# opendilab/DI-hpc

Measured on AMD Instinct MI355X. Metric: gae_fwd_bwd_samples_per_sec, higher is better.
Workload: dtype f32; 1 GPU; GAE fwd+bwd, T=1024, global B=65536 (65536 per GPU), fp32 (BASELINE.json configs[1]); T=1024, B_per_gpu=65536, global_B=65536, parallelism=batch-sharded x1, no data-path collective, launch=eager

## Files before the change

### di-hpc_amd/csrc/gae.hip

```cpp
#include <hip/hip_runtime.h>
#include <hip/hip_ext.h>

#include <atomic>
#include <initializer_list>
#include <new>
#include <type_traits>

#include "hostutil.hpp"
#include "hpc_rll_hip.h"
#include "wave.hpp"

namespace hpc_rll {
namespace {

__device__ __forceinline__ double geom_sum(double lam, int k) {
    if (k <= 0) return 0.0;
    if (lam == 1.0) return (double)k;
    if (lam > 0.0) return -expm1((double)k * log(lam)) / (1.0 - lam);
    return (1.0 - pow(lam, (double)k)) / (1.0 - lam);
}

__global__ void gae_coef_kernel(float* __restrict__ coef, int T, float gamma, float lambda) {
    const int t = blockIdx.x * blockDim.x + threadIdx.x;
    if (t >= T) return;
    const int k = T - t;
    const double lam = (double)lambda;
    coef[t] = (float)((double)gamma * lam * geom_sum(lam, k - 1) / geom_sum(lam, k));
}

template <int V, int LC, int NW, bool NTL, bool NTS, bool HALF = false>
__global__ __launch_bounds__(NW * 64) void gae_fwd_kernel(const float* __restrict__ value,
                                                          const float* __restrict__ reward,
                                                          float* __restrict__ adv,
                                                          const float* __restrict__ coef, int T, int B,
                                                          float gamma) {
    static_assert(!HALF || V == 1, "half-wave tiles hold one column per lane");
    constexpr int NWV = HALF ? 2 * NW : NW;
    constexpr int TILE = HALF ? 32 : 64 * V;
    __shared__ float lds[2 * NWV * TILE + 2 * NWV];
    float* const s_l0 = lds;
    float* const s_p0 = lds + 2 * NWV * TILE;

    const int lane = threadIdx.x & 63;
    const int wr = __builtin_amdgcn_readfirstlane((int)(threadIdx.x >> 6));
    const int cl = HALF ? (lane & 31) : lane;
    const int w = HALF ? 2 * wr + (lane >> 5) : wr;
    const long col = (long)blockIdx.x * TILE + (long)cl * V;
    const bool col_ok = col < (long)B;

    float carry[V];
#pragma unroll
    for (int k = 0; k < V; ++k) carry[k] = 0.f;

    constexpr int SPAN = NWV * LC;
    const int n_iter = (T + SPAN - 1) / SPAN;

    for (int it = 0; it < n_iter; ++it) {
        const int t1 = T - (it * NWV + (NWV - 1 - w)) * LC;
        const int t0 = t1 - LC;
        const int buf = it & 1;

        float L[LC][V];
        float P[LC];

        if (t0 >= 0) {
            Pack<V> vr[LC + 1], rr[LC];
            if (col_ok) {
                const float* vp = value + (size_t)t0 * B + col;
                const float* rp = reward + (size_t)t0 * B + col;
#pragma unroll
                for (int j = LC; j >= 0; --j) vr[j] = load_pack<V, NTL>(vp + (size_t)j * B);
#pragma unroll
                for (int j = LC - 1; j >= 0; --j) rr[j] = load_pack<V, NTL>(rp + (size_t)j * B);
            } else {
#pragma unroll
                for (int j = 0; j <= LC; ++j)
#pragma unroll
                    for (int k = 0; k < V; ++k) vr[j].v[k] = 0.f;
#pragma unroll
                for (int j = 0; j < LC; ++j)
#pragma unroll
                    for (int k = 0; k < V; ++k) rr[j].v[k] = 0.f;
            }
            float a[V];
#pragma unroll
            for (int k = 0; k < V; ++k) a[k] = 0.f;
            float p = 1.f;
#pragma unroll
            for (int j = LC - 1; j >= 0; --j) {
                const float c = coef[t0 + j];
#pragma unroll
                for (int k = 0; k < V; ++k) {
                    const float delta = fmaf(gamma, vr[j + 1].v[k], rr[j].v[k]) - vr[j].v[k];
                    a[k] = fmaf(c, a[k], delta);
                    L[j][k] = a[k];
                }
                p *= c;
                P[j] = p;
            }
        } else {
            float a[V];
#pragma unroll
            for (int k = 0; k < V; ++k) a[k] = 0.f;
            float p = 1.f;
#pragma unroll
            for (int j = LC - 1; j >= 0; --j) {
                const int t = t0 + j;
                if (t >= 0) {
                    const float c = coef[t];
                    Pack<V> v0, v1, r;
                    if (col_ok) {
                        v0 = load_pack<V, NTL>(value + (size_t)t * B + col);
                        v1 = load_pack<V, NTL>(value + (size_t)(t + 1) * B + col);
                        r = load_pack<V, NTL>(reward + (size_t)t * B + col);
                    } else {
#pragma unroll
                        for (int k = 0; k < V; ++k) v0.v[k] = v1.v[k] = r.v[k] = 0.f;
                    }
#pragma unroll
                    for (int k = 0; k < V; ++k) {
                        const float delta = fmaf(gamma, v1.v[k], r.v[k]) - v0.v[k];
                        a[k] = fmaf(c, a[k], delta);
                    }
                    p *= c;
                }
#pragma unroll
                for (int k = 0; k < V; ++k) L[j][k] = a[k];
                P[j] = p;
            }
        }

#pragma unroll
        for (int k = 0; k < V; ++k) s_l0[(buf * NWV + w) * TILE + cl * V + k] = L[0][k];
        if (cl == 0) s_p0[buf * NWV + w] = P[0];
        __syncthreads();

        float A[V], Aw[V];
#pragma unroll
        for (int k = 0; k < V; ++k) { A[k] = carry[k]; Aw[k] = 0.f; }
#pragma unroll
        for (int u = NWV - 1; u >= 0; --u) {
            if (u == w) {
#pragma unroll
                for (int k = 0; k < V; ++k) Aw[k] = A[k];
            }
            const float p0 = s_p0[buf * NWV + u];
#pragma unroll
            for (int k = 0; k < V; ++k) A[k] = fmaf(p0, A[k], s_l0[(buf * NWV + u) * TILE + cl * V + k]);
        }
#pragma unroll
        for (int k = 0; k < V; ++k) carry[k] = A[k];

        if (col_ok) {
#pragma unroll
            for (int j = LC - 1; j >= 0; --j) {
                const int t = t0 + j;
                if (t >= 0) {
                    Pack<V> o;
#pragma unroll
                    for (int k = 0; k < V; ++k) o.v[k] = fmaf(P[j], Aw[k], L[j][k]);
                    store_pack<V, NTS>(adv + (size_t)t * B + col, o);
                }
            }
        }
    }
}

template <int V, int LC, int NW, bool NTL, bool NTS, bool FULLB>
__global__ __launch_bounds__(NW * 64) void gae_fwd_pf_kernel(const float* __restrict__ value,
                                                             const float* __restrict__ reward,
                                                             float* __restrict__ adv,
                                                             const float* __restrict__ coef, int T, int B,
                                                             float gamma) {
    constexpr int TILE = 64 * V;
    __shared__ float lds[2 * NW * TILE + 2 * NW];
    float* const s_l0 = lds;
    float* const s_p0 = lds + 2 * NW * TILE;

    const int lane = threadIdx.x & 63;
    const int w = __builtin_amdgcn_readfirstlane((int)(threadIdx.x >> 6));
    const long col = (long)blockIdx.x * TILE + (long)lane * V;
    const bool col_ok = FULLB || col < (long)B;

    float carry[V];
#pragma unroll
    for (int k = 0; k < V; ++k) carry[k] = 0.f;

    constexpr int SPAN = NW * LC;
    const int n_full = T / SPAN;
    const bool ragged = (T % SPAN) != 0;

    Pack<V> vr[LC + 1], rr[LC];
#pragma unroll
    for (int j = 0; j <= LC; ++j)
#pragma unroll
        for (int k = 0; k < V; ++k) vr[j].v[k] = 0.f;
#pragma unroll
    for (int j = 0; j < LC; ++j)
#pragma unroll
        for (int k = 0; k < V; ++k) rr[j].v[k] = 0.f;

    auto chunk_t0 = [&](int it) { return T - (it * NW + (NW - 1 - w)) * LC - LC; };
    auto issue = [&](int it) {
        if (col_ok) {
            const int t0 = chunk_t0(it);
            const float* vp = value + (size_t)t0 * B + col;
            const float* rp = reward + (size_t)t0 * B + col;
#pragma unroll
            for (int j = LC; j >= 0; --j) vr[j] = load_pack<V, NTL>(vp + (size_t)j * B);
#pragma unroll
            for (int j = LC - 1; j >= 0; --j) rr[j] = load_pack<V, NTL>(rp + (size_t)j * B);
        }
    };
    auto finish = [&](auto guard_, int it, int t0, float (&L)[LC][V], float (&P)[LC]) {
        constexpr bool GUARD = decltype(guard_)::value != 0;
        const int buf = it & 1;
#pragma unroll
        for (int k = 0; k < V; ++k) s_l0[(buf * NW + w) * TILE + lane * V + k] = L[0][k];
        if (lane == 0) s_p0[buf * NW + w] = P[0];
        __syncthreads();
        float A[V], Aw[V];
#pragma unroll
        for (int k = 0; k < V; ++k) { A[k] = carry[k]; Aw[k] = 0.f; }
#pragma unroll
        for (int u = NW - 1; u >= 0; --u) {
            if (u == w) {
#pragma unroll
                for (int k = 0; k < V; ++k) Aw[k] = A[k];
            }
            const float p0 = s_p0[buf * NW + u];
#pragma unroll
            for (int k = 0; k < V; ++k) A[k] = fmaf(p0, A[k], s_l0[(buf * NW + u) * TILE + lane * V + k]);
        }
#pragma unroll
        for (int k = 0; k < V; ++k) carry[k] = A[k];
        if (col_ok) {
#pragma unroll
            for (int j = LC - 1; j >= 0; --j) {
                const int t = t0 + j;
                if (!GUARD || t >= 0) {
                    Pack<V> o;
#pragma unroll
                    for (int k = 0; k < V; ++k) o.v[k] = fmaf(P[j], Aw[k], L[j][k]);
                    store_pack<V, NTS>(adv + (size_t)t * B + col, o);
                }
            }
        }
    };

    if (n_full > 0) issue(0);
    for (int it = 0; it < n_full; ++it) {
        const int t0 = chunk_t0(it);
        float L[LC][V];
        float P[LC];
        {
            float a[V];
#pragma unroll
            for (int k = 0; k < V; ++k) a[k] = 0.f;
            float p = 1.f;
#pragma unroll
            for (int j = LC - 1; j >= 0; --j) {
                const float c = coef[t0 + j];
#pragma unroll
                for (int k = 0; k < V; ++k) {
                    const float delta = fmaf(gamma, vr[j + 1].v[k], rr[j].v[k]) - vr[j].v[k];
                    a[k] = fmaf(c, a[k], delta);
                    L[j][k] = a[k];
                }
                p *= c;
                P[j] = p;
            }
        }
        if (it + 1 < n_full) issue(it + 1);
        finish(std::integral_constant<int, 0>{}, it, t0, L, P);
    }
    if (ragged) {
        const int it = n_full;
        const int t0 = chunk_t0(it);
        float L[LC][V];
        float P[LC];
        float a[V];
#pragma unroll
        for (int k = 0; k < V; ++k) a[k] = 0.f;
        float p = 1.f;
#pragma unroll
        for (int j = LC - 1; j >= 0; --j) {
            const int t = t0 + j;
            if (t >= 0) {
                const float c = coef[t];
                Pack<V> v0, v1, r;
                if (col_ok) {
                    v0 = load_pack<V, NTL>(value + (size_t)t * B + col);
                    v1 = load_pack<V, NTL>(value + (size_t)(t + 1) * B + col);
                    r = load_pack<V, NTL>(reward + (size_t)t * B + col);
                } else {
#pragma unroll
                    for (int k = 0; k < V; ++k) v0.v[k] = v1.v[k] = r.v[k] = 0.f;
                }
#pragma unroll
                for (int k = 0; k < V; ++k) {
                    const float delta = fmaf(gamma, v1.v[k], r.v[k]) - v0.v[k];
                    a[k] = fmaf(c, a[k], delta);
                }
                p *= c;
            }
#pragma unroll
            for (int k = 0; k < V; ++k) L[j][k] = a[k];
            P[j] = p;
        }
        finish(std::integral_constant<int, 1>{}, it, t0, L, P);
    }
}

template <int V, int LC, int NW, bool NTL, bool NTS, bool HALF = false>
__global__ __launch_bounds__(NW * 64) void gae_bwd_kernel(const float* __restrict__ grad_adv,
                                                          float* __restrict__ grad_value,
                                                          float* __restrict__ grad_reward,
                                                          const float* __restrict__ coef, int T, int B,
                                                          float gamma) {
    static_assert(!HALF || V == 1, "half-wave tiles hold one column per lane");
    constexpr int NWV = HALF ? 2 * NW : NW;
    constexpr int TILE = HALF ? 32 : 64 * V;
    __shared__ float lds[2 * NWV * TILE + 2 * NWV];
    float* const s_l0 = lds;
    float* const s_p0 = lds + 2 * NWV * TILE;

    const int lane = threadIdx.x & 63;
    const int wr = __builtin_amdgcn_readfirstlane((int)(threadIdx.x >> 6));
    const int cl = HALF ? (lane & 31) : lane;
    const int w = HALF ? 2 * wr + (lane >> 5) : wr;
    const long col = (long)blockIdx.x * TILE + (long)cl * V;
    const bool col_ok = col < (long)B;

    float carry[V];
#pragma unroll
    for (int k = 0; k < V; ++k) carry[k] = 0.f;

    constexpr int SPAN = NWV * LC;
    const int n_iter = (T + SPAN - 1) / SPAN;

    for (int it = 0; it < n_iter; ++it) {
        const int t0 = (it * NWV + w) * LC;
        const int buf = it & 1;

        float L[LC][V];
        float Q[LC];
        {
            float a[V];
#pragma unroll
            for (int k = 0; k < V; ++k) a[k] = 0.f;
            float q = 1.f;
            if (t0 + LC <= T) {
                Pack<V> g[LC];
                if (col_ok) {
                    const float* gp = grad_adv + (size_t)t0 * B + col;
#pragma unroll
                    for (int j = 0; j < LC; ++j) g[j] = load_pack<V, NTL>(gp + (size_t)j * B);
                } else {
#pragma unroll
                    for (int j = 0; j < LC; ++j)
#pragma unroll
                        for (int k = 0; k < V; ++k) g[j].v[k] = 0.f;
                }
#pragma unroll
                for (int j = 0; j < LC; ++j) {
                    const int t = t0 + j;
                    const float c = (t > 0) ? coef[t - 1] : 0.f;
#pragma unroll
                    for (int k = 0; k < V; ++k) {
                        a[k] = fmaf(c, a[k], g[j].v[k]);
                        L[j][k] = a[k];
                    }
                    q *= c;
                    Q[j] = q;
                }
            } else {
#pragma unroll
                for (int j = 0; j < LC; ++j) {
                    const int t = t0 + j;
                    if (t < T) {
                        const float c = (t > 0) ? coef[t - 1] : 0.f;
                        Pack<V> g;
                        if (col_ok) {
                            g = load_pack<V, NTL>(grad_adv + (size_t)t * B + col);
                        } else {
#pragma unroll
                            for (int k = 0; k < V; ++k) g.v[k] = 0.f;
                        }
#pragma unroll
                        for (int k = 0; k < V; ++k) a[k] = fmaf(c, a[k], g.v[k]);
                        q *= c;
                    }
#pragma unroll
                    for (int k = 0; k < V; ++k) L[j][k] = a[k];
                    Q[j] = q;
                }
            }
        }

#pragma unroll
        for (int k = 0; k < V; ++k) s_l0[(buf * NWV + w) * TILE + cl * V + k] = L[LC - 1][k];
        if (cl == 0) s_p0[buf * NWV + w] = Q[LC - 1];
        __syncthreads();

        float A[V], Aw[V];
#pragma unroll
        for (int k = 0; k < V; ++k) { A[k] = carry[k]; Aw[k] = 0.f; }
#pragma unroll
        for (int u = 0; u < NWV; ++u) {
            if (u == w) {
#pragma unroll
                for (int k = 0; k < V; ++k) Aw[k] = A[k];
            }
            const float q0 = s_p0[buf * NWV + u];
#pragma unroll
            for (int k = 0; k < V; ++k) A[k] = fmaf(q0, A[k], s_l0[(buf * NWV + u) * TILE + cl * V + k]);
        }
#pragma unroll
        for (int k = 0; k < V; ++k) carry[k] = A[k];

        if (col_ok) {
            float prev[V];
#pragma unroll
            for (int k = 0; k < V; ++k) prev[k] = Aw[k];
#pragma unroll
            for (int j = 0; j < LC; ++j) {
                const int t = t0 + j;
                if (t < T) {
                    Pack<V> d, gv;
#pragma unroll
                    for (int k = 0; k < V; ++k) {
                        d.v[k] = fmaf(Q[j], Aw[k], L[j][k]);
                        gv.v[k] = fmaf(gamma, prev[k], -d.v[k]);
                        prev[k] = d.v[k];
                    }
                    if (grad_reward) store_pack<V, NTS>(grad_reward + (size_t)t * B + col, d);
                    if (grad_value) {
                        store_pack<V, NTS>(grad_value + (size_t)t * B + col, gv);
                        if (t == T - 1) {
                            Pack<V> last;
#pragma unroll
                            for (int k = 0; k < V; ++k) last.v[k] = gamma * d.v[k];
                            store_pack<V, NTS>(grad_value + (size_t)T * B + col, last);
                        }
                    }
                }
            }
        }
    }
}

template <int V, int LC, int NW, bool NTL, bool NTS, bool FULLB>
__global__ __launch_bounds__(NW * 64) void gae_bwd_pf_kernel(const float* __restrict__ grad_adv,
                                                             float* __restrict__ grad_value,
                                                             float* __restrict__ grad_reward,
                                                             const float* __restrict__ coef, int T, int B,
                                                             float gamma) {
    constexpr int TILE = 64 * V;
    __shared__ float lds[2 * NW * TILE + 2 * NW];
    float* const s_l0 = lds;
    float* const s_p0 = lds + 2 * NW * TILE;

    const int lane = threadIdx.x & 63;
    const int w = __builtin_amdgcn_readfirstlane((int)(threadIdx.x >> 6));
    const long col = (long)blockIdx.x * TILE + (long)lane * V;
    const bool col_ok = FULLB || col < (long)B;

    float carry[V];
#pragma unroll
    for (int k = 0; k < V; ++k) carry[k] = 0.f;

    constexpr int SPAN = NW * LC;
    const int n_full = T / SPAN;
    const bool ragged = (T % SPAN) != 0;

    Pack<V> g[LC];
#pragma unroll
    for (int j = 0; j < LC; ++j)
#pragma unroll
        for (int k = 0; k < V; ++k) g[j].v[k] = 0.f;

    auto chunk_t0 = [&](int it) { return (it * NW + w) * LC; };
    auto issue = [&](int it) {
        if (col_ok) {
            const float* gp = grad_adv + (size_t)chunk_t0(it) * B + col;
#pragma unroll
            for (int j = 0; j < LC; ++j) g[j] = load_pack<V, NTL>(gp + (size_t)j * B);
        }
    };
    auto finish = [&](auto guard_, int it, int t0, float (&L)[LC][V], float (&Q)[LC]) {
        constexpr bool GUARD = decltype(guard_)::value != 0;
        const int buf = it & 1;
#pragma unroll
        for (int k = 0; k < V; ++k) s_l0[(buf * NW + w) * TILE + lane * V + k] = L[LC - 1][k];
        if (lane == 0) s_p0[buf * NW + w] = Q[LC - 1];
        __syncthreads();
        float A[V], Aw[V];
#pragma unroll
        for (int k = 0; k < V; ++k) { A[k] = carry[k]; Aw[k] = 0.f; }
#pragma unroll
        for (int u = 0; u < NW; ++u) {
            if (u == w) {
#pragma unroll
                for (int k = 0; k < V; ++k) Aw[k] = A[k];
            }
            const float q0 = s_p0[buf * NW + u];
#pragma unroll
            for (int k = 0; k < V; ++k) A[k] = fmaf(q0, A[k], s_l0[(buf * NW + u) * TILE + lane * V + k]);
        }
#pragma unroll
        for (int k = 0; k < V; ++k) carry[k] = A[k];
        if (col_ok) {
            float prev[V];
#pragma unroll
            for (int k = 0; k < V; ++k) prev[k] = Aw[k];
#pragma unroll
            for (int j = 0; j < LC; ++j) {
                const int t = t0 + j;
                if (!GUARD || t < T) {
                    Pack<V> d, gv;
#pragma unroll
                    for (int k = 0; k < V; ++k) {
                        d.v[k] = fmaf(Q[j], Aw[k], L[j][k]);
                        gv.v[k] = fmaf(gamma, prev[k], -d.v[k]);
                        prev[k] = d.v[k];
                    }
                    store_pack<V, NTS>(grad_reward + (size_t)t * B + col, d);
                    store_pack<V, NTS>(grad_value + (size_t)t * B + col, gv);
                    if ((GUARD || j == LC - 1) && t == T - 1) {
                        Pack<V> last;
#pragma unroll
                        for (int k = 0; k < V; ++k) last.v[k] = gamma * d.v[k];
                        store_pack<V, NTS>(grad_value + (size_t)T * B + col, last);
                    }
                }
            }
        }
    };

    if (n_full > 0) issue(0);
    for (int it = 0; it < n_full; ++it) {
        const int t0 = chunk_t0(it);
        float L[LC][V];
        float Q[LC];
        {
            float a[V];
#pragma unroll
            for (int k = 0; k < V; ++k) a[k] = 0.f;
            float q = 1.f;
#pragma unroll
            for (int j = 0; j < LC; ++j) {
                const int t = t0 + j;
                const float c = (t > 0) ? coef[t - 1] : 0.f;
#pragma unroll
                for (int k = 0; k < V; ++k) {
                    a[k] = fmaf(c, a[k], g[j].v[k]);
                    L[j][k] = a[k];
                }
                q *= c;
                Q[j] = q;
            }
        }
        if (it + 1 < n_full) issue(it + 1);
        finish(std::integral_constant<int, 0>{}, it, t0, L, Q);
    }
    if (ragged) {
        const int it = n_full;
        const int t0 = chunk_t0(it);
        float L[LC][V];
        float Q[LC];
        float a[V];
#pragma unroll
        for (int k = 0; k < V; ++k) a[k] = 0.f;
        float q = 1.f;
#pragma unroll
        for (int j = 0; j < LC; ++j) {
            const int t = t0 + j;
            if (t < T) {
                const float c = (t > 0) ? coef[t - 1] : 0.f;
                Pack<V> gg;
                if (col_ok) {
                    gg = load_pack<V, NTL>(grad_adv + (size_t)t * B + col);
                } else {
#pragma unroll
                    for (int k = 0; k < V; ++k) gg.v[k] = 0.f;
                }
#pragma unroll
                for (int k = 0; k < V; ++k) a[k] = fmaf(c, a[k], gg.v[k]);
                q *= c;
            }
#pragma unroll
            for (int k = 0; k < V; ++k) L[j][k] = a[k];
            Q[j] = q;
        }
        finish(std::integral_constant<int, 1>{}, it, t0, L, Q);
    }
}

struct Cfg { int v, lc, nw, flags; bool half; bool pf; bool pf_refused; int plain_flags; };

struct KTime {
    bool on = false;
    int cap = 0, n = 0;
    hipEvent_t* ev = nullptr;
    int* kind = nullptr;
    std::atomic<int> last_cfg[2][6] = {};
};
KTime g_kt;

template <class K, class... A>
inline void launch(K kernel, dim3 grid, dim3 block, hipStream_t st, int kind, A... args) {
    if (g_kt.on && g_kt.n < g_kt.cap) {
        const int i = g_kt.n++;
        g_kt.kind[i] = kind;
        hipExtLaunchKernelGGL(kernel, grid, block, 0, st, g_kt.ev[2 * i], g_kt.ev[2 * i + 1], 0, args...);
    } else {
        hipLaunchKernelGGL(kernel, grid, block, 0, st, args...);
    }
}

inline int max_vec(int B, std::initializer_list<const void*> ptrs) {
    for (int v : {4, 2}) {
        bool ok = (B % v) == 0;
        for (const void* p : ptrs) ok = ok && aligned(p, 4 * v);
        if (ok) return v;
    }
    return 1;
}

inline Cfg choose_cfg(bool fwd, int T, int B, int vmax, int v, int lc, int nw, int flags) {
    auto wgs_for = [&](int vv) { return (B + 64 * vv - 1) / (64 * vv); };
    const bool all_auto = v == 0 && lc == 0 && nw == 0;
    const bool all_explicit = v != 0 && lc != 0 && nw != 0;
    const bool streaming = (12.0 * (double)T * (double)B) >= 300e6;
    int av, alc, anw, afl;
    bool apf = false;
    if (streaming && fwd) {
        av = (B >= 65536 && vmax >= 2) ? 2 : 1;
        const int wgs = wgs_for(av);
        if (wgs >= 1024) { alc = 16; anw = 8; }
        else if (wgs >= 512) { alc = 8; anw = av == 2 ? 2 : 4; }
        else { alc = 16; anw = 8; }
        afl = 3;
        if (vmax >= 2) {
            if (B < 65536) { if (B >= 32768) { av = 2; alc = 16; anw = 8; apf = true; } }
            else if (B < 131072) {
                if (vmax >= 4) { av = 4; alc = 4; anw = 8; } else { av = 2; alc = 4; anw = 4; }
                apf = true;
            }
            else if (B >= 262144) { av = 2; alc = 16; anw = 4; apf = true; }
        }
    } else if (streaming) {
        if (B >= 262144) { av = 1; alc = 8; anw = 8; apf = true; }
        else if (B >= 65536 && vmax >= 4) { av = 4; alc = 2; anw = 4; apf = true; }
        else if (B >= 131072 && vmax >= 2) { av = 2; alc = 2; anw = 4; }
        else if (B >= 65536 && vmax >= 2) { av = 2; alc = 2; anw = 4; }
        else if (B >= 32768 && vmax >= 4) { av = 4; alc = 4; anw = 4; apf = true; }
        else { av = 1; alc = 8; anw = 8; }
        afl = 2;
    } else {
        av = 1; alc = 16; anw = 4;
        while (anw < 16 && wgs_for(1) * anw < 2048) anw <<= 1;
        afl = 2;
        if (T >= 512 && wgs_for(1) >= 256 && anw == 8) {
            apf = true;
            if (!fwd) alc = 8;
        }
    }
    if (v == 0) v = av;
    if (v > vmax) v = vmax;
    if (lc == 0) {
        lc = alc;
        if (lc == 16 && v == 4) lc = 8;
    }
    if (nw == 0) {
        nw = anw;
        const int chunks = (T + lc - 1) / lc;
        while (nw > 1 && nw > chunks) nw >>= 1;
    }
    const int explicit_flags = flags;
    bool half = flags >= 0 && (flags & 4);
    if (flags < 0) {
        flags = afl;
        half = all_auto && !streaming && v == 1 && lc == 16 && nw == 16 && wgs_for(1) < 256 && T >= 512;
    }
    if (half && !(v == 1 && nw == 16 && (lc == 8 || lc == 16))) half = false;
    bool pf = !half && (explicit_flags >= 0 ? (explicit_flags & 8) != 0 : (all_auto && apf));
    if (pf && !(nw == 2 || nw == 4 || nw == 8)) pf = false;
    if (pf && fwd && !((lc == 4 || lc == 8 || lc == 16) && !(v == 4 && lc == 16) && !(v == 1 && lc == 4))) pf = false;
    if (pf && !fwd && !((lc == 2 || lc == 4 || lc == 8) && !(v == 1 && lc != 8))) pf = false;
    const int plain_flags = flags & 3;
    if (pf) flags |= 2;
    const bool pf_asked = explicit_flags >= 0 && (explicit_flags & 8) != 0;
    const bool pf_refused = pf_asked && (!all_explicit || (!half && !pf));
    Cfg out{v, lc, nw, flags & 3, half, pf, pf_refused, plain_flags};
    return out;
}

template <int N> using I = std::integral_constant<int, N>;

template <class F>
inline void for_each_cfg(F&& f) {
#define HPC_RLL_NW_ROW(V, LC) \
    f(I<V>{}, I<LC>{}, I<1>{}); f(I<V>{}, I<LC>{}, I<2>{}); f(I<V>{}, I<LC>{}, I<4>{}); \
    f(I<V>{}, I<LC>{}, I<8>{}); f(I<V>{}, I<LC>{}, I<16>{});
    HPC_RLL_NW_ROW(1, 4) HPC_RLL_NW_ROW(1, 8) HPC_RLL_NW_ROW(1, 16)
    HPC_RLL_NW_ROW(2, 2) HPC_RLL_NW_ROW(2, 4) HPC_RLL_NW_ROW(2, 8) HPC_RLL_NW_ROW(2, 16)
    HPC_RLL_NW_ROW(4, 2) HPC_RLL_NW_ROW(4, 4) HPC_RLL_NW_ROW(4, 8)
#undef HPC_RLL_NW_ROW
}

#define HPC_RLL_GAE_DISPATCH(KERNEL, KIND, ...)                                                    \
    do {                                                                                           \
        bool hit = false;                                                                          \
        {                                                                                          \
            std::atomic<int>* lc_ = g_kt.last_cfg[KIND];                                           \
            lc_[0] = cfg.v; lc_[1] = cfg.lc; lc_[2] = cfg.nw; lc_[3] = cfg.flags; lc_[4] = cfg.half; lc_[5] = cfg.pf; \
        }                                                                                          \
        if (cfg.half) {                                                                            \
            const dim3 grid((unsigned)((B + 31) / 32)), block(1024);                               \
            const bool ntl = cfg.flags & 1;                                                        \
            if (cfg.lc == 16) {                                                                    \
                if (ntl) launch(KERNEL<1, 16, 16, true, true, true>, grid, block, st, KIND, __VA_ARGS__);   \
                else launch(KERNEL<1, 16, 16, false, true, true>, grid, block, st, KIND, __VA_ARGS__);      \
            } else {                                                                               \
                if (ntl) launch(KERNEL<1, 8, 16, true, true, true>, grid, block, st, KIND, __VA_ARGS__);    \
                else launch(KERNEL<1, 8, 16, false, true, true>, grid, block, st, KIND, __VA_ARGS__);       \
            }                                                                                      \
            hit = true;                                                                            \
        }                                                                                          \
        auto go = [&](auto V_, auto LC_, auto NW_) {                                               \
            constexpr int V = decltype(V_)::value, LC = decltype(LC_)::value,                      \
                          NW = decltype(NW_)::value;                                               \
            if (!hit && cfg.v == V && cfg.lc == LC && cfg.nw == NW) {                                \
                const dim3 grid((unsigned)((B + 64 * V - 1) / (64 * V))), block(NW * 64);          \
                switch (cfg.flags) {                                                               \
                    case 0: launch(KERNEL<V, LC, NW, false, false>, grid, block, st, KIND, __VA_ARGS__); break; \
                    case 1: launch(KERNEL<V, LC, NW, true, false>, grid, block, st, KIND, __VA_ARGS__); break;  \
                    case 2: launch(KERNEL<V, LC, NW, false, true>, grid, block, st, KIND, __VA_ARGS__); break;  \
                    default: launch(KERNEL<V, LC, NW, true, true>, grid, block, st, KIND, __VA_ARGS__); break;  \
                }                                                                                  \
                hit = true;                                                                        \
            }                                                                                      \
        };                                                                                         \
        for_each_cfg(go);                                                                          \
        if (!hit) return HPC_RLL_EUNSUPPORTED;                                                     \
    } while (0)

template <class... A>
inline bool dispatch_fwd_pf(const Cfg& cfg, int B, hipStream_t st, A... args) {
    bool hit = false;
    auto go = [&](auto V_, auto LC_, auto NW_) {
        constexpr int V = decltype(V_)::value, LC = decltype(LC_)::value, NW = decltype(NW_)::value;
        if (!hit && cfg.v == V && cfg.lc == LC && cfg.nw == NW) {
            const dim3 grid((unsigned)((B + 64 * V - 1) / (64 * V))), block(NW * 64);
            const bool full = (B % (64 * V)) == 0;
            if (cfg.flags & 1) {
                if (full) launch(gae_fwd_pf_kernel<V, LC, NW, true, true, true>, grid, block, st, 0, args...);
                else launch(gae_fwd_pf_kernel<V, LC, NW, true, true, false>, grid, block, st, 0, args...);
            } else {
                if (full) launch(gae_fwd_pf_kernel<V, LC, NW, false, true, true>, grid, block, st, 0, args...);
                else launch(gae_fwd_pf_kernel<V, LC, NW, false, true, false>, grid, block, st, 0, args...);
            }
            hit = true;
        }
    };
#define HPC_RLL_PF_ROW(V, LC) go(I<V>{}, I<LC>{}, I<2>{}); go(I<V>{}, I<LC>{}, I<4>{}); go(I<V>{}, I<LC>{}, I<8>{});
    HPC_RLL_PF_ROW(1, 8) HPC_RLL_PF_ROW(1, 16) HPC_RLL_PF_ROW(2, 4) HPC_RLL_PF_ROW(2, 8) HPC_RLL_PF_ROW(2, 16)
    HPC_RLL_PF_ROW(4, 4) HPC_RLL_PF_ROW(4, 8)
#undef HPC_RLL_PF_ROW
    return hit;
}

template <class... A>
inline bool dispatch_bwd_pf(const Cfg& cfg, int B, hipStream_t st, A... args) {
    bool hit = false;
    auto go = [&](auto V_, auto LC_, auto NW_) {
        constexpr int V = decltype(V_)::value, LC = decltype(LC_)::value, NW = decltype(NW_)::value;
        if (!hit && cfg.v == V && cfg.lc == LC && cfg.nw == NW) {
            const dim3 grid((unsigned)((B + 64 * V - 1) / (64 * V))), block(NW * 64);
            const bool full = (B % (64 * V)) == 0;
            if (cfg.flags & 1) {
                if (full) launch(gae_bwd_pf_kernel<V, LC, NW, true, true, true>, grid, block, st, 1, args...);
                else launch(gae_bwd_pf_kernel<V, LC, NW, true, true, false>, grid, block, st, 1, args...);
            } else {
                if (full) launch(gae_bwd_pf_kernel<V, LC, NW, false, true, true>, grid, block, st, 1, args...);
                else launch(gae_bwd_pf_kernel<V, LC, NW, false, true, false>, grid, block, st, 1, args...);
            }
            hit = true;
        }
    };
#define HPC_RLL_PF_ROW(V, LC) go(I<V>{}, I<LC>{}, I<2>{}); go(I<V>{}, I<LC>{}, I<4>{}); go(I<V>{}, I<LC>{}, I<8>{});
    HPC_RLL_PF_ROW(1, 8) HPC_RLL_PF_ROW(2, 2) HPC_RLL_PF_ROW(2, 4) HPC_RLL_PF_ROW(2, 8)
    HPC_RLL_PF_ROW(4, 2) HPC_RLL_PF_ROW(4, 4) HPC_RLL_PF_ROW(4, 8)
#undef HPC_RLL_PF_ROW
    return hit;
}

inline int check_launch() {
    const hipError_t e = hipGetLastError();
    return e == hipSuccess ? HPC_RLL_OK : (int)e;
}

}
}

using namespace hpc_rll;

extern "C" int hpc_rll_gae_coef(float* coef, int T, float gamma, float lambda, void* stream) {
    if (T < 0) return HPC_RLL_EINVAL;
    if (T == 0) return HPC_RLL_OK;
    if (!coef) return HPC_RLL_EINVAL;
    hipLaunchKernelGGL(gae_coef_kernel, dim3((T + 255) / 256), dim3(256), 0, (hipStream_t)stream, coef, T, gamma,
                       lambda);
    return check_launch();
}

extern "C" int hpc_rll_gae_forward_ex(const float* value, const float* reward, float* adv, const float* coef,
                                      int T, int B, float gamma, int vec, int lc, int nw, int flags, void* stream) {
    if (T < 0 || B < 0) return HPC_RLL_EINVAL;
    if (T == 0 || B == 0) return HPC_RLL_OK;
    if (!value || !reward || !adv || !coef) return HPC_RLL_EINVAL;
    if (!aligned(value, 4) || !aligned(reward, 4) || !aligned(adv, 4) || !aligned(coef, 4)) return HPC_RLL_EALIGN;
    if (flags >= 0 && (flags & ~15)) return HPC_RLL_EUNSUPPORTED;
    const Cfg cfg = choose_cfg(true, T, B, max_vec(B, {value, reward, adv}), vec, lc, nw, flags);
    if (cfg.pf_refused) return HPC_RLL_EUNSUPPORTED;
    hipStream_t st = (hipStream_t)stream;
    if (cfg.pf) {
        std::atomic<int>* lc_ = g_kt.last_cfg[0];
        lc_[0] = cfg.v; lc_[1] = cfg.lc; lc_[2] = cfg.nw; lc_[3] = cfg.flags; lc_[4] = 0; lc_[5] = 1;
        if (!dispatch_fwd_pf(cfg, B, st, value, reward, adv, coef, T, B, gamma)) return HPC_RLL_EUNSUPPORTED;
        return check_launch();
    }
    HPC_RLL_GAE_DISPATCH(gae_fwd_kernel, 0, value, reward, adv, coef, T, B, gamma);
    return check_launch();
}

extern "C" int hpc_rll_gae_forward(const float* value, const float* reward, float* adv, const float* coef, int T,
                                   int B, float gamma, void* stream) {
    return hpc_rll_gae_forward_ex(value, reward, adv, coef, T, B, gamma, 0, 0, 0, -1, stream);
}

extern "C" int hpc_rll_gae_backward_ex(const float* grad_adv, float* grad_value, float* grad_reward,
                                       const float* coef, int T, int B, float gamma, int vec, int lc, int nw,
                                       int flags, void* stream) {
    if (T < 0 || B < 0) return HPC_RLL_EINVAL;
    if (B == 0) return HPC_RLL_OK;
    if (T == 0) {
        if (grad_value) return (int)hipMemsetAsync(grad_value, 0, sizeof(float) * (size_t)B, (hipStream_t)stream);
        return HPC_RLL_OK;
    }
    if (!grad_adv || !coef) return HPC_RLL_EINVAL;
    if (!grad_value && !grad_reward) return HPC_RLL_OK;
    if (!aligned(grad_adv, 4) || !aligned(grad_value, 4) || !aligned(grad_reward, 4) || !aligned(coef, 4))
        return HPC_RLL_EALIGN;
    if (flags >= 0 && (flags & ~15)) return HPC_RLL_EUNSUPPORTED;
    Cfg cfg = choose_cfg(false, T, B, max_vec(B, {grad_adv, grad_value, grad_reward}), vec, lc, nw, flags);
    if (cfg.pf_refused) return HPC_RLL_EUNSUPPORTED;
    if (cfg.pf && (!grad_value || !grad_reward)) {
        cfg.pf = false;
        cfg.flags = cfg.plain_flags;
    }
    hipStream_t st = (hipStream_t)stream;
    if (cfg.pf) {
        std::atomic<int>* lc_ = g_kt.last_cfg[1];
        lc_[0] = cfg.v; lc_[1] = cfg.lc; lc_[2] = cfg.nw; lc_[3] = cfg.flags; lc_[4] = 0; lc_[5] = 1;
        if (!dispatch_bwd_pf(cfg, B, st, grad_adv, grad_value, grad_reward, coef, T, B, gamma)) return HPC_RLL_EUNSUPPORTED;
        return check_launch();
    }
    HPC_RLL_GAE_DISPATCH(gae_bwd_kernel, 1, grad_adv, grad_value, grad_reward, coef, T, B, gamma);
    return check_launch();
}

extern "C" int hpc_rll_gae_backward(const float* grad_adv, float* grad_value, float* grad_reward, const float* coef,
                                    int T, int B, float gamma, void* stream) {
    return hpc_rll_gae_backward_ex(grad_adv, grad_value, grad_reward, coef, T, B, gamma, 0, 0, 0, -1, stream);
}

extern "C" int hpc_rll_ktime_begin(int capacity) {
    if (capacity <= 0 || g_kt.on) return HPC_RLL_EINVAL;
    g_kt.ev = new (std::nothrow) hipEvent_t[2 * (size_t)capacity];
    g_kt.kind = new (std::nothrow) int[capacity];
    hipError_t e = (g_kt.ev && g_kt.kind) ? hipSuccess : hipErrorOutOfMemory;
    int made = 0;
    for (; e == hipSuccess && made < 2 * capacity; ++made) e = hipEventCreate(&g_kt.ev[made]);
    if (e != hipSuccess) {
        for (int i = 0; i + 1 < made; ++i) (void)hipEventDestroy(g_kt.ev[i]);
        delete[] g_kt.ev;
        delete[] g_kt.kind;
        g_kt.ev = nullptr;
        g_kt.kind = nullptr;
        g_kt.cap = g_kt.n = 0;
        return (int)e;
    }
    g_kt.cap = capacity;
    g_kt.n = 0;
    g_kt.on = true;
    return HPC_RLL_OK;
}

extern "C" int hpc_rll_ktime_end(float* ms, int* kind, int max) {
    if (!g_kt.on) return HPC_RLL_EINVAL;
    g_kt.on = false;
    const int n = g_kt.n;
    int rc = n;
    for (int i = 0; i < n; ++i) {
        hipError_t e = hipEventSynchronize(g_kt.ev[2 * i + 1]);
        float t = 0.f;
        if (e == hipSuccess) e = hipEventElapsedTime(&t, g_kt.ev[2 * i], g_kt.ev[2 * i + 1]);
        if (e != hipSuccess) { rc = (int)e > 0 ? -1000 - (int)e : HPC_RLL_EINVAL; break; }
        if (i < max) {
            if (ms) ms[i] = t;
            if (kind) kind[i] = g_kt.kind[i];
        }
    }
    for (int i = 0; i < 2 * g_kt.cap; ++i) (void)hipEventDestroy(g_kt.ev[i]);
    delete[] g_kt.ev;
    delete[] g_kt.kind;
    g_kt.ev = nullptr;
    g_kt.kind = nullptr;
    g_kt.cap = g_kt.n = 0;
    return rc;
}

extern "C" int hpc_rll_gae_last_config(int dir, int* out) {
    if ((dir != 0 && dir != 1) || !out) return HPC_RLL_EINVAL;
    for (int i = 0; i < 6; ++i) out[i] = g_kt.last_cfg[dir][i];
    return HPC_RLL_OK;
}
```

Before: 278.8 billion samples/s.

## Add half-wave tiling to prefetching GAE kernels and route half configs through them

Adds a HALF template mode to the prefetching forward and backward GAE kernels. Each 64-lane wavefront is split into two 32-column virtual waves, so a 16-wave block covers 32 columns with 32 time chunks. The config chooser now enables the prefetch path for the existing half-wave configuration (v=1, lc=16, nw=16), which previously ran only the plain kernel, and new launchers dispatch the half variants. This aims to bring software-pipelined loads to the half-wave schedule chosen for small grids. The cost is a longer cross-chunk LDS scan over twice as many virtual waves, and the forward path is limited to B divisible by 32.

```diff
diff --git a/di-hpc_amd/csrc/gae.hip b/di-hpc_amd/csrc/gae.hip
--- a/di-hpc_amd/csrc/gae.hip
+++ b/di-hpc_amd/csrc/gae.hip
@@ -166,27 +166,31 @@
     }
 }
 
-template <int V, int LC, int NW, bool NTL, bool NTS, bool FULLB>
+template <int V, int LC, int NW, bool NTL, bool NTS, bool FULLB, bool HALF = false>
 __global__ __launch_bounds__(NW * 64) void gae_fwd_pf_kernel(const float* __restrict__ value,
                                                              const float* __restrict__ reward,
                                                              float* __restrict__ adv,
                                                              const float* __restrict__ coef, int T, int B,
                                                              float gamma) {
-    constexpr int TILE = 64 * V;
-    __shared__ float lds[2 * NW * TILE + 2 * NW];
+    static_assert(!HALF || V == 1, "half-wave tiles hold one column per lane");
+    constexpr int NWV = HALF ? 2 * NW : NW;
+    constexpr int TILE = HALF ? 32 : 64 * V;
+    __shared__ float lds[2 * NWV * TILE + 2 * NWV];
     float* const s_l0 = lds;
-    float* const s_p0 = lds + 2 * NW * TILE;
+    float* const s_p0 = lds + 2 * NWV * TILE;
 
     const int lane = threadIdx.x & 63;
-    const int w = __builtin_amdgcn_readfirstlane((int)(threadIdx.x >> 6));
-    const long col = (long)blockIdx.x * TILE + (long)lane * V;
+    const int wr = __builtin_amdgcn_readfirstlane((int)(threadIdx.x >> 6));
+    const int cl = HALF ? (lane & 31) : lane;
+    const int w = HALF ? 2 * wr + (lane >> 5) : wr;
+    const long col = (long)blockIdx.x * TILE + (long)cl * V;
     const bool col_ok = FULLB || col < (long)B;
 
     float carry[V];
 #pragma unroll
     for (int k = 0; k < V; ++k) carry[k] = 0.f;
 
-    constexpr int SPAN = NW * LC;
+    constexpr int SPAN = NWV * LC;
     const int n_full = T / SPAN;
     const bool ragged = (T % SPAN) != 0;
 
@@ -200,7 +204,7 @@
 #pragma unroll
         for (int k = 0; k < V; ++k) rr[j].v[k] = 0.f;
 
-    auto chunk_t0 = [&](int it) { return T - (it * NW + (NW - 1 - w)) * LC - LC; };
+    auto chunk_t0 = [&](int it) { return T - (it * NWV + (NWV - 1 - w)) * LC - LC; };
     auto issue = [&](int it) {
         if (col_ok) {
             const int t0 = chunk_t0(it);
@@ -216,21 +220,21 @@
         constexpr bool GUARD = decltype(guard_)::value != 0;
         const int buf = it & 1;
 #pragma unroll
-        for (int k = 0; k < V; ++k) s_l0[(buf * NW + w) * TILE + lane * V + k] = L[0][k];
-        if (lane == 0) s_p0[buf * NW + w] = P[0];
+        for (int k = 0; k < V; ++k) s_l0[(buf * NWV + w) * TILE + cl * V + k] = L[0][k];
+        if (cl == 0) s_p0[buf * NWV + w] = P[0];
         __syncthreads();
         float A[V], Aw[V];
 #pragma unroll
         for (int k = 0; k < V; ++k) { A[k] = carry[k]; Aw[k] = 0.f; }
 #pragma unroll
-        for (int u = NW - 1; u >= 0; --u) {
+        for (int u = NWV - 1; u >= 0; --u) {
             if (u == w) {
 #pragma unroll
                 for (int k = 0; k < V; ++k) Aw[k] = A[k];
             }
-            const float p0 = s_p0[buf * NW + u];
-#pragma unroll
-            for (int k = 0; k < V; ++k) A[k] = fmaf(p0, A[k], s_l0[(buf * NW + u) * TILE + lane * V + k]);
+            const float p0 = s_p0[buf * NWV + u];
+#pragma unroll
+            for (int k = 0; k < V; ++k) A[k] = fmaf(p0, A[k], s_l0[(buf * NWV + u) * TILE + cl * V + k]);
         }
 #pragma unroll
         for (int k = 0; k < V; ++k) carry[k] = A[k];
@@ -450,27 +454,31 @@
     }
 }
 
-template <int V, int LC, int NW, bool NTL, bool NTS, bool FULLB>
+template <int V, int LC, int NW, bool NTL, bool NTS, bool FULLB, bool HALF = false>
 __global__ __launch_bounds__(NW * 64) void gae_bwd_pf_kernel(const float* __restrict__ grad_adv,
                                                              float* __restrict__ grad_value,
                                                              float* __restrict__ grad_reward,
                                                              const float* __restrict__ coef, int T, int B,
                                                              float gamma) {
-    constexpr int TILE = 64 * V;
-    __shared__ float lds[2 * NW * TILE + 2 * NW];
+    static_assert(!HALF || V == 1, "half-wave tiles hold one column per lane");
+    constexpr int NWV = HALF ? 2 * NW : NW;
+    constexpr int TILE = HALF ? 32 : 64 * V;
+    __shared__ float lds[2 * NWV * TILE + 2 * NWV];
     float* const s_l0 = lds;
-    float* const s_p0 = lds + 2 * NW * TILE;
+    float* const s_p0 = lds + 2 * NWV * TILE;
 
     const int lane = threadIdx.x & 63;
-    const int w = __builtin_amdgcn_readfirstlane((int)(threadIdx.x >> 6));
-    const long col = (long)blockIdx.x * TILE + (long)lane * V;
+    const int wr = __builtin_amdgcn_readfirstlane((int)(threadIdx.x >> 6));
+    const int cl = HALF ? (lane & 31) : lane;
+    const int w = HALF ? 2 * wr + (lane >> 5) : wr;
+    const long col = (long)blockIdx.x * TILE + (long)cl * V;
     const bool col_ok = FULLB || col < (long)B;
 
     float carry[V];
 #pragma unroll
     for (int k = 0; k < V; ++k) carry[k] = 0.f;
 
-    constexpr int SPAN = NW * LC;
+    constexpr int SPAN = NWV * LC;
     const int n_full = T / SPAN;
     const bool ragged = (T % SPAN) != 0;
 
@@ -480,7 +488,7 @@
 #pragma unroll
         for (int k = 0; k < V; ++k) g[j].v[k] = 0.f;
 
-    auto chunk_t0 = [&](int it) { return (it * NW + w) * LC; };
+    auto chunk_t0 = [&](int it) { return (it * NWV + w) * LC; };
     auto issue = [&](int it) {
         if (col_ok) {
             const float* gp = grad_adv + (size_t)chunk_t0(it) * B + col;
@@ -492,21 +500,21 @@
         constexpr bool GUARD = decltype(guard_)::value != 0;
         const int buf = it & 1;
 #pragma unroll
-        for (int k = 0; k < V; ++k) s_l0[(buf * NW + w) * TILE + lane * V + k] = L[LC - 1][k];
-        if (lane == 0) s_p0[buf * NW + w] = Q[LC - 1];
+        for (int k = 0; k < V; ++k) s_l0[(buf * NWV + w) * TILE + cl * V + k] = L[LC - 1][k];
+        if (cl == 0) s_p0[buf * NWV + w] = Q[LC - 1];
         __syncthreads();
         float A[V], Aw[V];
 #pragma unroll
         for (int k = 0; k < V; ++k) { A[k] = carry[k]; Aw[k] = 0.f; }
 #pragma unroll
-        for (int u = 0; u < NW; ++u) {
+        for (int u = 0; u < NWV; ++u) {
             if (u == w) {
 #pragma unroll
                 for (int k = 0; k < V; ++k) Aw[k] = A[k];
             }
-            const float q0 = s_p0[buf * NW + u];
-#pragma unroll
-            for (int k = 0; k < V; ++k) A[k] = fmaf(q0, A[k], s_l0[(buf * NW + u) * TILE + lane * V + k]);
+            const float q0 = s_p0[buf * NWV + u];
+#pragma unroll
+            for (int k = 0; k < V; ++k) A[k] = fmaf(q0, A[k], s_l0[(buf * NWV + u) * TILE + cl * V + k]);
         }
 #pragma unroll
         for (int k = 0; k < V; ++k) carry[k] = A[k];
@@ -685,10 +693,12 @@
         half = all_auto && !streaming && v == 1 && lc == 16 && nw == 16 && wgs_for(1) < 256 && T >= 512;
     }
     if (half && !(v == 1 && nw == 16 && (lc == 8 || lc == 16))) half = false;
-    bool pf = !half && (explicit_flags >= 0 ? (explicit_flags & 8) != 0 : (all_auto && apf));
-    if (pf && !(nw == 2 || nw == 4 || nw == 8)) pf = false;
-    if (pf && fwd && !((lc == 4 || lc == 8 || lc == 16) && !(v == 4 && lc == 16) && !(v == 1 && lc == 4))) pf = false;
-    if (pf && !fwd && !((lc == 2 || lc == 4 || lc == 8) && !(v == 1 && lc != 8))) pf = false;
+    const bool half_pf = half && lc == 16 && (!fwd || B % 32 == 0) &&
+                         (explicit_flags >= 0 ? (explicit_flags & 8) != 0 : all_auto);
+    bool pf = half_pf || (!half && (explicit_flags >= 0 ? (explicit_flags & 8) != 0 : (all_auto && apf)));
+    if (pf && !half && !(nw == 2 || nw == 4 || nw == 8)) pf = false;
+    if (pf && !half && fwd && !((lc == 4 || lc == 8 || lc == 16) && !(v == 4 && lc == 16) && !(v == 1 && lc == 4))) pf = false;
+    if (pf && !half && !fwd && !((lc == 2 || lc == 4 || lc == 8) && !(v == 1 && lc != 8))) pf = false;
     const int plain_flags = flags & 3;
     if (pf) flags |= 2;
     const bool pf_asked = explicit_flags >= 0 && (explicit_flags & 8) != 0;
@@ -797,6 +807,26 @@
     return hit;
 }
 
+template <class... A>
+inline void launch_fwd_half_pf(const Cfg& cfg, int B, hipStream_t st, A... args) {
+    const dim3 grid((unsigned)(B / 32)), block(1024);
+    if (cfg.flags & 1) launch(gae_fwd_pf_kernel<1, 16, 16, true, true, true, true>, grid, block, st, 0, args...);
+    else launch(gae_fwd_pf_kernel<1, 16, 16, false, true, true, true>, grid, block, st, 0, args...);
+}
+
+template <class... A>
+inline void launch_bwd_half_pf(const Cfg& cfg, int B, hipStream_t st, A... args) {
+    const dim3 grid((unsigned)((B + 31) / 32)), block(1024);
+    const bool full = (B % 32) == 0;
+    if (cfg.flags & 1) {
+        if (full) launch(gae_bwd_pf_kernel<1, 16, 16, true, true, true, true>, grid, block, st, 1, args...);
+        else launch(gae_bwd_pf_kernel<1, 16, 16, true, true, false, true>, grid, block, st, 1, args...);
+    } else {
+        if (full) launch(gae_bwd_pf_kernel<1, 16, 16, false, true, true, true>, grid, block, st, 1, args...);
+        else launch(gae_bwd_pf_kernel<1, 16, 16, false, true, false, true>, grid, block, st, 1, args...);
+    }
+}
+
 inline int check_launch() {
     const hipError_t e = hipGetLastError();
     return e == hipSuccess ? HPC_RLL_OK : (int)e;
@@ -828,8 +858,9 @@
     hipStream_t st = (hipStream_t)stream;
     if (cfg.pf) {
         std::atomic<int>* lc_ = g_kt.last_cfg[0];
-        lc_[0] = cfg.v; lc_[1] = cfg.lc; lc_[2] = cfg.nw; lc_[3] = cfg.flags; lc_[4] = 0; lc_[5] = 1;
-        if (!dispatch_fwd_pf(cfg, B, st, value, reward, adv, coef, T, B, gamma)) return HPC_RLL_EUNSUPPORTED;
+        lc_[0] = cfg.v; lc_[1] = cfg.lc; lc_[2] = cfg.nw; lc_[3] = cfg.flags; lc_[4] = cfg.half; lc_[5] = 1;
+        if (cfg.half) launch_fwd_half_pf(cfg, B, st, value, reward, adv, coef, T, B, gamma);
+        else if (!dispatch_fwd_pf(cfg, B, st, value, reward, adv, coef, T, B, gamma)) return HPC_RLL_EUNSUPPORTED;
         return check_launch();
     }
     HPC_RLL_GAE_DISPATCH(gae_fwd_kernel, 0, value, reward, adv, coef, T, B, gamma);
@@ -864,8 +895,9 @@
     hipStream_t st = (hipStream_t)stream;
     if (cfg.pf) {
         std::atomic<int>* lc_ = g_kt.last_cfg[1];
-        lc_[0] = cfg.v; lc_[1] = cfg.lc; lc_[2] = cfg.nw; lc_[3] = cfg.flags; lc_[4] = 0; lc_[5] = 1;
-        if (!dispatch_bwd_pf(cfg, B, st, grad_adv, grad_value, grad_reward, coef, T, B, gamma)) return HPC_RLL_EUNSUPPORTED;
+        lc_[0] = cfg.v; lc_[1] = cfg.lc; lc_[2] = cfg.nw; lc_[3] = cfg.flags; lc_[4] = cfg.half; lc_[5] = 1;
+        if (cfg.half) launch_bwd_half_pf(cfg, B, st, grad_adv, grad_value, grad_reward, coef, T, B, gamma);
+        else if (!dispatch_bwd_pf(cfg, B, st, grad_adv, grad_value, grad_reward, coef, T, B, gamma)) return HPC_RLL_EUNSUPPORTED;
         return check_launch();
     }
     HPC_RLL_GAE_DISPATCH(gae_bwd_kernel, 1, grad_adv, grad_value, grad_reward, coef, T, B, gamma);
```

Result: no change. 278.5 billion samples/s (-0.1%).
